# qwagrox/field-coverage-path-planning

Measured on AMD Instinct MI355X. Metric: validated path points/sec (Clothoid+speed+geofence) on 500x200m field batch, higher is better.
Workload: dtype f64; 1 GPU; cfg1 x 4096: 4096 fields of 500 x 200 m per GPU, ARC turns (the reference's own model, pinned to its outputs) at the reference's sampling, 1691 points per field; a step = one fresh plan call of the ba; turn_model=arc (reference, pinned), points_per_gpu_step=6926336, fields_per_gpu=4096, setup=device

## Files before the change

### field_coverage_path_planning_amd/csrc/fcpp_quiet_fn.h

```cpp
#pragma once
#include "fcpp_pointfn.h"

namespace fcpp {

#ifndef FCPP_DENSE_NT
#define FCPP_DENSE_NT 0
#endif
typedef double st_pair_f64 __attribute__((ext_vector_type(2), aligned(8)));
typedef uint32_t st_pair_u32 __attribute__((ext_vector_type(2), aligned(4)));
template <bool NT>
__device__ __forceinline__ void st2(double *ptr, double a, double b)
{
    st_pair_f64 v = { a, b };
    if (NT) __builtin_nontemporal_store(v, reinterpret_cast<st_pair_f64 *>(ptr));
    else *reinterpret_cast<st_pair_f64 *>(ptr) = v;
}
template <bool NT>
__device__ __forceinline__ void st2(uint32_t *ptr, uint32_t a, uint32_t b)
{
    st_pair_u32 v = { a, b };
    if (NT) __builtin_nontemporal_store(v, reinterpret_cast<st_pair_u32 *>(ptr));
    else *reinterpret_cast<st_pair_u32 *>(ptr) = v;
}
template <bool NT>
__device__ __forceinline__ void store_pair(bool has0, bool has1, int64_t g, double px0, double px1, double py0, double py1, double k0,
                                           double k1, double v, uint32_t f0, uint32_t f1, double *__restrict__ xo,
                                           double *__restrict__ yo, double *__restrict__ ko, double *__restrict__ vo,
                                           uint32_t *__restrict__ fso)
{
    if (has0 && has1) {
        st2<NT>(xo + g, px0, px1);
        st2<NT>(yo + g, py0, py1);
        st2<NT>(ko + g, k0, k1);
        st2<NT>(vo + g, v, v);
        st2<NT>(fso + g, f0, f1);
    } else if (has0) {
        xo[g] = px0; yo[g] = py0; ko[g] = k0; vo[g] = v; fso[g] = f0;
    } else if (has1) {
        xo[g + 1] = px1; yo[g + 1] = py1; ko[g + 1] = k1; vo[g + 1] = v; fso[g + 1] = f1;
    }
}

__device__ __forceinline__ double line_start_curvature(const DevField &q, const DevConst &cst, int idx, double &jump_len)
{
    const int per = q.n_line + q.n_turn;
    double tx, ty, x0, y0, x1, y1;
    uint32_t fw;
    eval_main(q, cst, idx - 1, per - 1, tx, ty, fw);
    eval_main(q, cst, idx, 0, x0, y0, fw);
    eval_main(q, cst, idx, 1, x1, y1, fw);
    const double dx1 = x0 - tx, dy1 = y0 - ty, dx2 = x1 - x0, dy2 = y1 - y0;
    jump_len = seg_len(dx1, dy1);
    return curv_chords(dx1, dy1, jump_len, dx2, dy2, seg_len(dx2, dy2));
}

__device__ __forceinline__ void stage_turn_template(const DevConst &cst, double *__restrict__ tmpl_lds)
{
    const int lane = threadIdx.x & 63;
    if (lane < cst.tmpl_n) {
        const double2 t = cst.tmpl_u[lane];
        tmpl_lds[lane] = t.x; tmpl_lds[TMPL_LDS + lane] = t.y; tmpl_lds[2 * TMPL_LDS + lane] = cst.tmpl_u_dk[lane].y;
    }
    wave_sync();
}

template <int KINDS, bool STAGED, bool OBS>
__device__ __forceinline__ void quiet_tile(const DevTile &tl, const DevField *__restrict__ fg, const DevPrim *__restrict__ prims,
                                           const DevConst &cst, const DevObstacles &obs, double *my_lds ,
                                           double *__restrict__ tmpl_lds ,
                                           double *__restrict__ xo, double *__restrict__ yo, double *__restrict__ ko,
                                           double *__restrict__ vo, uint32_t *__restrict__ fso,
                                           unsigned long long *sink_outside, unsigned long long *sink_obstacle)
{
    const int lane = threadIdx.x & 63;
    const DevField &q = *fg;
    const int cnt = tl.count;
    const int64_t g0 = q.pt_off + tl.start;
    const int odd = (int)(g0 & 1);
    constexpr bool NT = FCPP_DENSE_NT && KINDS != 16;
    const double ntol = -cst.geofence_tol;
    auto outside = [&](double px, double py) -> bool {
        bool out = false;
#pragma unroll
        for (int e = 0; e < 4; ++e) out = out | (q.ex[e] * px + q.ey[e] * py + q.eo[e] < ntol);
        return out;
    };
    int nout = 0, nobs = 0;
    if ((KINDS & 16) && (KINDS == 16 || tl.quiet == 4)) {
        int per = q.n_line + q.n_turn, nl = q.n_line, last = q.n_turn - 1, n_pass = q.P, idx_base = tl.idx0;
        int rev = q.reverse_order, sfr = q.start_from_right, rotated = q.rotated;
        const bool arc = q.turn_model == FCPP_TURN_ARC;
        double xr = arc ? q.max_x : (q.max_x - q.R), xl = arc ? q.min_x : (q.min_x + q.R);
        double k_last = cst.turn_kappa_last[q.reverse_order ? 1 : 0];
        double k_start = cst.field_junc[tl.field].x;
        double min_y = q.min_y, Wd = q.W, lstep = q.line_step, lex = q.lex, lsx = q.lsx;
        double rc = q.rot_cos, rs = q.rot_sin, rcx = q.rot_cx, rcy = q.rot_cy;
        double v_work = cst.v_work, v_turn = cst.v_turn;
        double e0x = q.ex[0], e0y = q.ey[0], e0o = q.eo[0], e1x = q.ex[1], e1y = q.ey[1], e1o = q.eo[1];
        double e2x = q.ex[2], e2y = q.ey[2], e2o = q.eo[2], e3x = q.ex[3], e3y = q.ey[3], e3o = q.eo[3];
        double ntl = ntol;
        int n_obs = q.obs_count;
        const bool fence = q.span_inside == 0;
        FCPP_PIN(per); FCPP_PIN(nl); FCPP_PIN(last); FCPP_PIN(n_pass); FCPP_PIN(idx_base); FCPP_PIN(rev); FCPP_PIN(sfr); FCPP_PIN(rotated);
        FCPP_PIN(xr); FCPP_PIN(xl); FCPP_PIN(k_last); FCPP_PIN(k_start); FCPP_PIN(min_y); FCPP_PIN(Wd); FCPP_PIN(lstep); FCPP_PIN(lex); FCPP_PIN(lsx);
        FCPP_PIN(v_work); FCPP_PIN(v_turn); FCPP_PIN(n_obs);
        FCPP_PIN_V(rc); FCPP_PIN_V(rs); FCPP_PIN_V(rcx); FCPP_PIN_V(rcy);
        FCPP_PIN_V(e0x); FCPP_PIN_V(e0y); FCPP_PIN_V(e0o); FCPP_PIN_V(e1x); FCPP_PIN_V(e1y); FCPP_PIN_V(e1o);
        FCPP_PIN_V(e2x); FCPP_PIN_V(e2y); FCPP_PIN_V(e2o); FCPP_PIN_V(e3x); FCPP_PIN_V(e3y); FCPP_PIN_V(e3o); FCPP_PIN_V(ntl);
        auto outside_s = [&](double px, double py) -> bool {
            return (e0x * px + e0y * py + e0o < ntl) | (e1x * px + e1y * py + e1o < ntl) | (e2x * px + e2y * py + e2o < ntl) |
                   (e3x * px + e3y * py + e3o < ntl);
        };
        auto sample = [&](int dq, int off, double &px, double &py, double &kp, double &v, uint32_t &fw) {
            const int idx = idx_base + dq;
            const int pi = rev ? (n_pass - 1 - idx) : idx;
            const double y = min_y + (double)pi * Wd;
            const bool go_left = sfr ? ((idx & 1) == 0) : ((idx & 1) == 1);
            if (off < nl) {
                px = go_left ? ((double)off * -lstep + lex) : ((double)off * lstep + lsx);
                if (off == nl - 1) px = go_left ? lsx : lex;
                py = y;
                kp = (off == 0 && idx > 0) ? k_start : 0.0;
                v = v_work;
                fw = FCPP_KIND_SWATH | ((uint32_t)pi << FCPP_INDEX_SHIFT);
            } else {
                const int c = off - nl;
                double tx, ty, tk;
                if (STAGED) { tx = tmpl_lds[c]; ty = tmpl_lds[TMPL_LDS + c]; tk = tmpl_lds[2 * TMPL_LDS + c]; }
                else { const double2 t = cst.tmpl_u[c]; tx = t.x; ty = t.y; tk = cst.tmpl_u_dk[c].y; }
                const bool turn_right = !go_left;
                px = arc ? (turn_right ? (xr - tx) : (xl + tx)) : (turn_right ? (xr + tx) : (xl - tx));
                py = y + ty;
                kp = c == last ? k_last : tk;
                v = v_turn;
                fw = FCPP_KIND_UTURN | ((uint32_t)pi << FCPP_INDEX_SHIFT);
            }
            if (rotated) {
                const double tx = px - rcx, ty = py - rcy;
                px = (tx * rc - ty * rs) + rcx;
                py = (tx * rs + ty * rc) + rcy;
            }
        };
        const unsigned uper = (unsigned)per, step_q = 128u / uper, step_r = 128u - step_q * uper;
        const unsigned a1 = (unsigned)(tl.off0 + 2 * lane - odd + 1);
        int dq1 = (int)(a1 / uper), off1 = (int)(a1 - (unsigned)dq1 * uper);
#pragma unroll
        for (int k = 0; k < TILE_POINTS / 128; ++k) {
            if (k > 0 && 128 * k - odd >= cnt) break;
            const int j = 2 * (lane + 64 * k) - odd;
            const bool has0 = j >= 0 && j < cnt, has1 = j + 1 < cnt;
            double px0, py0, k0, v0, px1, py1, k1, v1;
            uint32_t f0, f1;
            const int dq0 = off1 == 0 ? dq1 - 1 : dq1, off0 = off1 == 0 ? per - 1 : off1 - 1;
            sample(dq0, off0, px0, py0, k0, v0, f0);
            sample(dq1, off1, px1, py1, k1, v1, f1);
            off1 += (int)step_r; dq1 += (int)step_q;
            if (off1 >= per) { off1 -= per; ++dq1; }
            if (fence) {
                const bool o0 = has0 && outside_s(px0, py0), o1 = has1 && outside_s(px1, py1);
                nout += (o0 ? 1 : 0) + (o1 ? 1 : 0);
                f0 |= o0 ? FCPP_FLAG_OUTSIDE : 0u;
                f1 |= o1 ? FCPP_FLAG_OUTSIDE : 0u;
            }
            if (OBS && n_obs > 0) {
                double mnx = has0 ? px0 : (has1 ? px1 : FCPP_INF), mxx = has0 ? px0 : (has1 ? px1 : -FCPP_INF);
                double mny = has0 ? py0 : (has1 ? py1 : FCPP_INF), mxy = has0 ? py0 : (has1 ? py1 : -FCPP_INF);
                if (has1) { mnx = fmin(mnx, px1); mxx = fmax(mxx, px1); mny = fmin(mny, py1); mxy = fmax(mxy, py1); }
#pragma unroll
                for (int o = 32; o > 0; o >>= 1) {
                    mnx = fmin(mnx, __shfl_xor(mnx, o)); mny = fmin(mny, __shfl_xor(mny, o));
                    mxx = fmax(mxx, __shfl_xor(mxx, o)); mxy = fmax(mxy, __shfl_xor(mxy, o));
                }
                const double ox[2] = { has0 ? px0 : px1, px1 }, oy[2] = { has0 ? py0 : py1, py1 };
                const unsigned m = obstacle_mask<2>(obs, q.obs_first, q.obs_first + q.obs_count, my_lds, mnx, mny, mxx, mxy, ox, oy,
                                                    has1 ? 2 : (has0 ? 1 : 0));
                const bool b0 = has0 && (m & 1u), b1 = has1 && (m & 2u);
                nobs += (b0 ? 1 : 0) + (b1 ? 1 : 0);
                f0 |= b0 ? FCPP_FLAG_OBSTACLE : 0u;
                f1 |= b1 ? FCPP_FLAG_OBSTACLE : 0u;
            }
            const int64_t g = g0 + j;
            if (has0 && has1) {
                st2<NT>(xo + g, px0, px1);
                st2<NT>(yo + g, py0, py1);
                st2<NT>(ko + g, k0, k1);
                st2<NT>(vo + g, v0, v1);
                st2<NT>(fso + g, f0, f1);
            } else if (has0) {
                xo[g] = px0; yo[g] = py0; ko[g] = k0; vo[g] = v0; fso[g] = f0;
            } else if (has1) {
                xo[g + 1] = px1; yo[g + 1] = py1; ko[g + 1] = k1; vo[g + 1] = v1; fso[g + 1] = f1;
            }
        }
    } else if ((KINDS & 8) && (KINDS == 8 || tl.quiet == 3)) {
        const int idx = tl.idx0;
        const int pi = q.reverse_order ? (q.P - 1 - idx) : idx;
        const double y = q.min_y + (double)pi * q.W;
        const bool go_left = q.start_from_right ? ((idx & 1) == 0) : ((idx & 1) == 1);
        const bool turn_right = !go_left, arc = q.turn_model == FCPP_TURN_ARC;
        const double xr = arc ? q.max_x : (q.max_x - q.R), xl = arc ? q.min_x : (q.min_x + q.R);
        const uint32_t fw = FCPP_KIND_UTURN | ((uint32_t)pi << FCPP_INDEX_SHIFT);
        const double k_last = cst.turn_kappa_last[q.reverse_order ? 1 : 0];
        const int last = q.n_turn - 1;
        auto sample = [&](int tk, double &px, double &py, double &kp) {
            const int c = min(max(tk, 0), last);
            const double2 t = cst.tmpl_u[c];
            px = arc ? (turn_right ? (xr - t.x) : (xl + t.x)) : (turn_right ? (xr + t.x) : (xl - t.x));
            py = y + t.y;
            if (q.rotated) rotate_back(q, px, py);
            kp = c == last ? k_last : cst.tmpl_u_dk[c].y;
        };
#pragma unroll
        for (int k = 0; k < TILE_POINTS / 128; ++k) {
            if (k > 0 && 128 * k - odd >= cnt) break;
            const int j = 2 * (lane + 64 * k) - odd;
            const bool has0 = j >= 0 && j < cnt, has1 = j + 1 < cnt;
            double px0, py0, k0, px1, py1, k1;
            sample(tl.off0 + j, px0, py0, k0);
            sample(tl.off0 + j + 1, px1, py1, k1);
            uint32_t f0 = fw, f1 = fw;
            const bool o0 = has0 && outside(px0, py0), o1 = has1 && outside(px1, py1);
            nout += (o0 ? 1 : 0) + (o1 ? 1 : 0);
            f0 |= o0 ? FCPP_FLAG_OUTSIDE : 0u;
            f1 |= o1 ? FCPP_FLAG_OUTSIDE : 0u;
            if (OBS && q.obs_count > 0) {
                double mnx = has0 ? px0 : (has1 ? px1 : FCPP_INF), mxx = has0 ? px0 : (has1 ? px1 : -FCPP_INF);
                double mny = has0 ? py0 : (has1 ? py1 : FCPP_INF), mxy = has0 ? py0 : (has1 ? py1 : -FCPP_INF);
                if (has1) { mnx = fmin(mnx, px1); mxx = fmax(mxx, px1); mny = fmin(mny, py1); mxy = fmax(mxy, py1); }
#pragma unroll
                for (int o = 32; o > 0; o >>= 1) {
                    mnx = fmin(mnx, __shfl_xor(mnx, o)); mny = fmin(mny, __shfl_xor(mny, o));
                    mxx = fmax(mxx, __shfl_xor(mxx, o)); mxy = fmax(mxy, __shfl_xor(mxy, o));
                }
                const double ox[2] = { has0 ? px0 : px1, px1 }, oy[2] = { has0 ? py0 : py1, py1 };
                const unsigned m = obstacle_mask<2>(obs, q.obs_first, q.obs_first + q.obs_count, my_lds, mnx, mny, mxx, mxy, ox, oy,
                                                    has1 ? 2 : (has0 ? 1 : 0));
                const bool b0 = has0 && (m & 1u), b1 = has1 && (m & 2u);
                nobs += (b0 ? 1 : 0) + (b1 ? 1 : 0);
                f0 |= b0 ? FCPP_FLAG_OBSTACLE : 0u;
                f1 |= b1 ? FCPP_FLAG_OBSTACLE : 0u;
            }
            store_pair<NT>(has0, has1, g0 + j, px0, px1, py0, py1, k0, k1, cst.v_turn, f0, f1, xo, yo, ko, vo, fso);
        }
    } else if (KINDS & 6) {
        double ax, ay, sx, sy, bx, by, vnom;
        int n_lin;
        uint32_t fw;
        bool rot;
        if (tl.quiet == 1) {
            const int idx = tl.idx0;
            const int pi = q.reverse_order ? (q.P - 1 - idx) : idx;
            const bool go_left = q.start_from_right ? ((idx & 1) == 0) : ((idx & 1) == 1);
            ax = go_left ? q.lex : q.lsx; bx = go_left ? q.lsx : q.lex; sx = go_left ? -q.line_step : q.line_step;
            ay = by = q.min_y + (double)pi * q.W; sy = 0.0;
            n_lin = q.n_line;
            rot = q.rotated != 0;
            fw = FCPP_KIND_SWATH | ((uint32_t)pi << FCPP_INDEX_SHIFT);
            vnom = cst.v_work;
        } else {
            const DevPrim &p = prims[tl.idx0];
            ax = p.a[0]; ay = p.a[1]; bx = p.a[2]; by = p.a[3]; sx = p.a[4]; sy = p.a[5];
            n_lin = p.n;
            rot = false;
            fw = p.fs; vnom = p.v_nom;
        }
        auto lin = [&](int r, double &px, double &py) {
            px = (double)r * sx + ax; py = (double)r * sy + ay;
            if (r == n_lin - 1) { px = bx; py = by; }
        };
        const bool has_start = tl.quiet == 1 && tl.off0 == 0 && tl.idx0 > 0;
        const double k_start = has_start ? cst.field_junc[tl.field].x : 0.0;
        double ex0, ey0, ex1, ey1;
        lin(tl.off0, ex0, ey0);
        lin(tl.off0 + cnt - 1, ex1, ey1);
        if (rot) { rotate_back(q, ex0, ey0); rotate_back(q, ex1, ey1); }
        const bool ends_out = outside(ex0, ey0) || outside(ex1, ey1);
        const double bminx = fmin(ex0, ex1), bmaxx = fmax(ex0, ex1), bminy = fmin(ey0, ey1), bmaxy = fmax(ey0, ey1);
#pragma unroll
        for (int k = 0; k < TILE_POINTS / 128; ++k) {
            if (k > 0 && 128 * k - odd >= cnt) break;
            const int j = 2 * (lane + 64 * k) - odd;
            const bool has0 = j >= 0 && j < cnt, has1 = j + 1 < cnt;
            double px0, py0, px1, py1;
            lin(tl.off0 + j, px0, py0);
            lin(tl.off0 + j + 1, px1, py1);
            if (rot) { rotate_back(q, px0, py0); rotate_back(q, px1, py1); }
            uint32_t f0 = fw, f1 = fw;
            if (ends_out) {
                const bool o0 = has0 && outside(px0, py0), o1 = has1 && outside(px1, py1);
                nout += (o0 ? 1 : 0) + (o1 ? 1 : 0);
                f0 |= o0 ? FCPP_FLAG_OUTSIDE : 0u;
                f1 |= o1 ? FCPP_FLAG_OUTSIDE : 0u;
            }
            if (OBS && q.obs_count > 0) {
                const double ox[2] = { has0 ? px0 : px1, px1 }, oy[2] = { has0 ? py0 : py1, py1 };
                const unsigned m = obstacle_mask<2>(obs, q.obs_first, q.obs_first + q.obs_count, my_lds, bminx, bminy, bmaxx, bmaxy,
                                                    ox, oy, has1 ? 2 : (has0 ? 1 : 0));
                const bool b0 = has0 && (m & 1u), b1 = has1 && (m & 2u);
                nobs += (b0 ? 1 : 0) + (b1 ? 1 : 0);
                f0 |= b0 ? FCPP_FLAG_OBSTACLE : 0u;
                f1 |= b1 ? FCPP_FLAG_OBSTACLE : 0u;
            }
            const double k0 = (has_start && j == 0) ? k_start : 0.0, k1 = (has_start && j + 1 == 0) ? k_start : 0.0;
            store_pair<NT>(has0, has1, g0 + j, px0, px1, py0, py1, k0, k1, vnom, f0, f1, xo, yo, ko, vo, fso);
        }
    }
    if (__ballot(nout | nobs)) {
        const long long io = wave_sum_i(nout), ib = wave_sum_i(nobs);
        if (lane == 0 && io) atomicAdd(sink_outside, (unsigned long long)io);
        if (lane == 0 && ib) atomicAdd(sink_obstacle, (unsigned long long)ib);
    }
}

struct FieldStatView {
    int n_line, n_turn, reverse_order;
    double line_step;
    int64_t n_main;
    double2 junc;
    __device__ __forceinline__ void set(const DevField &q, double2 j) { n_line = q.n_line; n_turn = q.n_turn; reverse_order = q.reverse_order; line_step = q.line_step; n_main = q.n_main; junc = j; }
    __device__ __forceinline__ void load(const DevField *__restrict__ fields, const DevConst &cst, int64_t field)
    {
        const DevField &q = fields[field];
        n_line = q.n_line; n_turn = q.n_turn; reverse_order = q.reverse_order; line_step = q.line_step; n_main = q.n_main;
        junc = cst.field_junc ? cst.field_junc[field] : make_double2(0.0, 0.0);
    }
};

__device__ __forceinline__ TilePartial quiet_run_partial(const DevRun &run, const DevTile &tl, const FieldStatView &q,
                                                         const DevPrim *__restrict__ prims, const DevConst &cst)
{
    TilePartial tp;
    tp.main_len = tp.main_time_pre = tp.main_time = tp.head_len = tp.head_time_pre = tp.head_time = 0.0;
    tp.max_kappa = tp.max_alat = tp.max_jump = 0.0;
    tp.n_viol = 0; tp.n_outside = 0; tp.n_in_obstacle = 0; tp.n_adjusted = 0;
    if (tl.quiet == 4) {
        const bool rv = q.reverse_order != 0;
        const double tmk = rv ? cst.turn_max_kappa[1] : cst.turn_max_kappa[0], tmj = rv ? cst.turn_max_jump[1] : cst.turn_max_jump[0];
        const double tkl = rv ? cst.turn_kappa_last[1] : cst.turn_kappa_last[0];
        const int per = q.n_line + q.n_turn;
        const double n_pass = (double)(run.count / per), n_jump = n_pass - (tl.idx0 == 0 ? 1.0 : 0.0);
        const double line_len = (double)(q.n_line - 1) * fabs(q.line_step);
        const double2 junc = q.junc;
        const double jl = n_jump > 0.0 ? junc.y : 0.0, k0 = n_jump > 0.0 ? junc.x : 0.0;
        tp.main_len = n_pass * (line_len + cst.turn_len) + n_jump * jl;
        tp.main_time_pre = tp.main_time = n_pass * (line_len / fmax(cst.ms_work, 0.1) + cst.turn_time) +
                                          n_jump * (jl / fmax(((cst.v_turn + cst.v_work) / 2) / 3.6, 0.1));
        tp.max_kappa = fmax(tmk, k0);
        tp.max_alat = fmax(cst.ms_turn * cst.ms_turn * tmk, cst.ms_work * cst.ms_work * k0);
        tp.max_jump = fmax(tmj, n_jump > 0.0 ? fmax(fabs(k0 - tkl), k0) : 0.0);
    } else     if (tl.quiet == 3) {
        const bool rv = q.reverse_order != 0;
        const double tmk = rv ? cst.turn_max_kappa[1] : cst.turn_max_kappa[0];
        tp.main_len = cst.turn_len; tp.main_time_pre = tp.main_time = cst.turn_time;
        tp.max_kappa = tmk; tp.max_alat = cst.ms_turn * cst.ms_turn * tmk;
        tp.max_jump = rv ? cst.turn_max_jump[1] : cst.turn_max_jump[0];
    } else {
        double step_len, msnom;
        int layer;
        if (tl.quiet == 1) { step_len = fabs(q.line_step); msnom = cst.ms_work; layer = 0; }
        else {
            const DevPrim &p = prims[tl.idx0];
            const double sx = p.a[4], sy = p.a[5];
            step_len = (sy == 0.0) ? fabs(sx) : ((sx == 0.0) ? fabs(sy) : sqrt(sx * sx + sy * sy));
            msnom = nominal_ms(p.fs, cst); layer = tl.start >= q.n_main ? 1 : 0;
        }
        const bool at_line_start = tl.quiet == 1 && tl.off0 == 0;
        double len = (double)(at_line_start ? run.count - 1 : run.count) * step_len, t = len / fmax(msnom, 0.1);
        if (at_line_start && tl.idx0 > 0) {
            const double k0 = q.junc.x, jl = q.junc.y;
            len += jl;
            t += jl / fmax(((cst.v_turn + cst.v_work) / 2) / 3.6, 0.1);
            tp.max_kappa = k0; tp.max_alat = cst.ms_work * cst.ms_work * k0;
            tp.max_jump = fmax(fabs(k0 - (q.reverse_order ? cst.turn_kappa_last[1] : cst.turn_kappa_last[0])), k0);
        }
        tp.main_len = layer ? 0.0 : len; tp.main_time_pre = layer ? 0.0 : t; tp.main_time = layer ? 0.0 : t;
        tp.head_len = layer ? len : 0.0; tp.head_time_pre = layer ? t : 0.0; tp.head_time = layer ? t : 0.0;
    }
    return tp;
}

}
```

### field_coverage_path_planning_amd/csrc/fcpp_sparse.hip

```cpp
#include "fcpp_sparse2_fn.h"
#include "fcpp_quiet_fn.h"
#include "fcpp_devplan.h"

namespace fcpp {

template <int SP_WAVES, int PTS>
__global__ __launch_bounds__(64 * SP_WAVES) void k_plan_sparse(const DevWaveTile *__restrict__ wtiles, const int32_t *__restrict__ ids, int64_t n_wtiles,
                                                               const DevField *__restrict__ fields, const DevPrim *__restrict__ prims,
                                                               DevConst cst, DevObstacles obs, double *__restrict__ xo, double *__restrict__ yo,
                                                               double *__restrict__ ko, double *__restrict__ vo, uint32_t *__restrict__ fso,
                                                               TilePartial *__restrict__ partial, int xcd_map)
{
    __shared__ double obs_lds[SP_WAVES][2 * OBS_LDS_VERTS];
    __shared__ double atab[ATAN_TAB_DOUBLES];
    __shared__ double plds[SP_WAVES][TILE_PRIMS_LDS];
    const int wave = __builtin_amdgcn_readfirstlane((int)(threadIdx.x >> 6)), lane = threadIdx.x & 63;
    const unsigned bid = xcd_map ? (blockIdx.x & 7u) * (gridDim.x >> 3) + (blockIdx.x >> 3) : blockIdx.x;
    const int64_t slot = (int64_t)bid * SP_WAVES + wave;
    if (slot >= n_wtiles) return;
    atan_tab_stage(atab);
    const DevWaveTile wt = wtiles[ids ? (int64_t)ids[slot] : slot];
    SparseAcc acc;
    acc.clear();
    sparse_tile2<false>(wt, fields[wt.field], prims, cst, obs, obs_lds[wave], atab, plds[wave], xo, yo, ko, vo, fso, acc);

    double g[3] = { 0.0, 0.0, 0.0 };
    const int out0 = wt.hb, out1 = wt.hb + wt.count;
    if (out0 < wt.rel_seam) g[0] = wave4_to_hi<0>(acc.s_len[0], acc.s_tpre[0], acc.s_t[0], 0.0);
    if (out1 > wt.rel_seam + 1) g[1] = wave4_to_hi<0>(acc.s_len[1], acc.s_tpre[1], acc.s_t[1], 0.0);
    if (__ballot(acc.mk != 0.0 || acc.mj != 0.0) != 0ull) g[2] = wave4_to_hi<1>(acc.mk, acc.ma, acc.mj, 0.0);
    const int vs = WAVE4_SLOT(lane);
    if (lane >= 60 && vs < 3) {
        double *tp = reinterpret_cast<double *>(&partial[wt.tile]);
        tp[vs] = g[0]; tp[3 + vs] = g[1]; tp[6 + vs] = g[2];
    }
    if (lane == 63) {
        TilePartial &tp = partial[wt.tile];
        tp.n_viol = acc.c_viol; tp.n_outside = acc.c_out; tp.n_in_obstacle = acc.c_obs; tp.n_adjusted = acc.c_adj;
    }
}

template <int W, bool OBS>
__device__ __forceinline__ void field_span_chunk(const DevFieldPack &pk, int wave, const DevConst &cst, const DevObstacles &obs, double *obs_lds,
                                                 double *tlds, double *__restrict__ xo, double *__restrict__ yo, double *__restrict__ ko,
                                                 double *__restrict__ vo, uint32_t *__restrict__ fso, unsigned long long *cnt)
{
    static_assert(W == FUSED_SPAN_CHUNKS, "one chunk per wavefront");
    const int64_t S = pk.span_points;
    const DevField &f = pk.field;
    const unsigned per = (unsigned)(f.n_line + f.n_turn);
    const int r0 = (int)(f.pt_off & (TILE_POINTS - 1));
    const int c_first = (int)(S < TILE_POINTS - r0 ? S : TILE_POINTS - r0);
    const int n_chunks = (int)((r0 + S + TILE_POINTS - 1) / TILE_POINTS);
    if (wave >= n_chunks) return;
    wave_sync();
    stage_turn_template(cst, tlds);
    DevTile tl;
    const unsigned start = wave == 0 ? 0u : (unsigned)(c_first + (wave - 1) * TILE_POINTS);
    tl.field = pk.work.field; tl.start = start; tl.quiet = 4; tl.stat_tile = 0;
    tl.count = wave == 0 ? c_first : (int)((S - start < TILE_POINTS) ? S - start : TILE_POINTS);
    tl.idx0 = __builtin_amdgcn_readfirstlane((int)(start / per)); tl.off0 = __builtin_amdgcn_readfirstlane((int)(start - (unsigned)tl.idx0 * per));
    tl.count = __builtin_amdgcn_readfirstlane(tl.count);
    quiet_tile<16, true, OBS>(tl, &f, nullptr, cst, obs, obs_lds, tlds, xo, yo, ko, vo, fso, cnt, cnt + 1);
}

struct DirectRule {
    int64_t n = 0, gen = 0;
    const int64_t *plan_totals = nullptr, *agg = nullptr;
};
template <int W, bool OBS, bool SPANS, bool DIRECT = false>
__device__ __forceinline__ void plan_sparse_fields_body(const DevFieldPack *__restrict__ packs,
                                                              DevConst cst, double *__restrict__ xo, double *__restrict__ yo,
                                                              double *__restrict__ ko, double *__restrict__ vo, uint32_t *__restrict__ fso,
                                                              DevObstacles obs, TilePartial *__restrict__ partial,
                                                              const TilePartial *__restrict__ totals, fcpp_field_stats *__restrict__ stats,
                                                              const DirectRule rule = DirectRule())
{
    __shared__ double obs_lds[W][OBS ? 2 * OBS_LDS_VERTS : 1];
    __shared__ TilePartial red[FIELD_WORK_TILES];
    __shared__ double atab[ATAN_TAB_DOUBLES];
    static_assert(3 * TMPL_LDS >= TILE_PRIMS_LDS, "one area serves both phases");
    __shared__ double wlds[W][3 * TMPL_LDS];
    __shared__ unsigned long long span_cnt[W][2];
    const int wave = __builtin_amdgcn_readfirstlane((int)(threadIdx.x >> 6)), lane = threadIdx.x & 63;
    atan_tab_stage(atab);
    const unsigned wg = DIRECT ? blockIdx.x - 1u : blockIdx.x;
    const DevFieldPack &pk = packs[wg];
    const DevFieldWork w = pk.work;
    if (DIRECT) {
        int64_t flag[PF_COUNT];
#pragma unroll
        for (int k = 0; k < PF_COUNT; ++k) flag[k] = rule.plan_totals[PC_COLS + k];
        const int nblk = (int)offset_blocks(rule.n);
        const int64_t a_work = offset_total_part(rule.agg, nblk, PC_WORK, lane), a_unf = offset_total_part(rule.agg, nblk, PC_UNFUSABLE, lane),
                      a_wsp = offset_total_part(rule.agg, nblk, PC_WORK_SPAN_PTS, lane);
        bool ok = off_wave_sum(a_work) == rule.n && off_wave_sum(a_unf) == 0 && off_wave_sum(a_wsp) > 0;
#pragma unroll
        for (int k = 0; k < PF_COUNT; ++k) ok = ok && flag[k] != rule.gen;
        if (!ok || w.n_tiles < 0) return;
        __builtin_amdgcn_sched_barrier(0);
    }
#ifdef FCPP_DIAG_SPARSE
    if (g_sparse_stop == -2) return;
#endif
    auto plan_tile = [&](const int t) {
        const DevWaveTile wt = pk.tile[t];
        SparseAcc acc;
        acc.clear();
        sparse_tile2<true>(wt, pk.field, pk.prims[t], cst, obs, obs_lds[wave], atab, wlds[wave], xo, yo, ko, vo, fso, acc);
        double g[3] = { 0.0, 0.0, 0.0 };
        const int out0 = wt.hb, out1 = wt.hb + wt.count;
        if (out0 < wt.rel_seam) g[0] = wave4_to_hi<0>(acc.s_len[0], acc.s_tpre[0], acc.s_t[0], 0.0);
        if (out1 > wt.rel_seam + 1) g[1] = wave4_to_hi<0>(acc.s_len[1], acc.s_tpre[1], acc.s_t[1], 0.0);
        if (__ballot(acc.mk != 0.0 || acc.mj != 0.0) != 0ull) g[2] = wave4_to_hi<1>(acc.mk, acc.ma, acc.mj, 0.0);
        const int vs = WAVE4_SLOT(lane);
        if (lane >= 60 && vs < 3) {
            double *tp = reinterpret_cast<double *>(&red[t]);
            tp[vs] = g[0]; tp[3 + vs] = g[1]; tp[6 + vs] = g[2];
        }
        if (lane == 63) { red[t].n_viol = acc.c_viol; red[t].n_outside = acc.c_out; red[t].n_in_obstacle = acc.c_obs; red[t].n_adjusted = acc.c_adj; }
    };
    if (lane < 2) span_cnt[wave][lane] = 0;
    auto span_phase = [&]() {
        const DevFieldPack *pk2 = &pk;
        asm volatile("" : "+s"(pk2) : : "memory");
        if (pk2->span_points > 0) field_span_chunk<W, OBS>(*pk2, wave, cst, obs, obs_lds[wave], wlds[wave], xo, yo, ko, vo, fso, &span_cnt[wave][0]);
    };
    if (wave < w.n_tiles) plan_tile(wave);
    if (SPANS) span_phase();
    static_assert(sizeof(TilePartial) == 13 * 8 && sizeof(fcpp_field_stats) == 13 * 8, "statistics records are thirteen 8-byte components");
    unsigned long long run_v = 0, c_out = 0, c_obs = 0;
    if (wave == 0) {
        if (lane < 13) run_v = reinterpret_cast<const unsigned long long *>(&totals[wg])[lane];
        if (!DIRECT && lane < w.n_entries) { const TilePartial &slot = partial[w.e_first + lane]; c_out = (unsigned long long)slot.n_outside; c_obs = (unsigned long long)slot.n_in_obstacle; }
    }
    asm volatile("s_waitcnt lgkmcnt(0)\n\ts_barrier" ::: "memory");
    if (wave != 0) return;
    if (!DIRECT && (c_out | c_obs) != 0ull) { partial[w.e_first + lane].n_outside = 0; partial[w.e_first + lane].n_in_obstacle = 0; }
    if (lane < W) { c_out += span_cnt[lane][0]; c_obs += span_cnt[lane][1]; }
    if (__ballot((c_out | c_obs) != 0ull) != 0ull) {
#pragma unroll
        for (int o = FIELD_WORK_ENTRIES / 2; o > 0; o >>= 1) { c_out += __shfl_xor(c_out, o); c_obs += __shfl_xor(c_obs, o); }
    }
    if (lane >= 13) return;
    const unsigned long long *rv = reinterpret_cast<const unsigned long long *>(red) + lane;
    unsigned long long bits;
    if (lane < 9) {
        double a = __longlong_as_double((long long)run_v);
        for (int t = 0; t < w.n_tiles; ++t) {
            const double x = __longlong_as_double((long long)rv[13 * t]);
            a = lane < 6 ? a + x : max_raw(a, x);
        }
        bits = (unsigned long long)__double_as_longlong(a);
    } else {
        bits = run_v;
        for (int t = 0; t < w.n_tiles; ++t) bits += rv[13 * t];
        if (lane == 10) bits += c_out;
        if (lane == 11) bits += c_obs;
    }
    reinterpret_cast<unsigned long long *>(&stats[w.field])[lane] = bits;
}

template <int W, bool OBS, bool SPANS>
__global__ __launch_bounds__(64 * W) void k_plan_sparse_fields(const DevFieldPack *__restrict__ packs, DevConst cst, double *__restrict__ xo, double *__restrict__ yo,
                                                              double *__restrict__ ko, double *__restrict__ vo, uint32_t *__restrict__ fso,
                                                              DevObstacles obs, TilePartial *__restrict__ partial,
                                                              const TilePartial *__restrict__ totals, fcpp_field_stats *__restrict__ stats)
{
    plan_sparse_fields_body<W, OBS, SPANS>(packs, cst, xo, yo, ko, vo, fso, obs, partial, totals, stats);
}

template <int W>
__global__ __launch_bounds__(64 * W) void k_plan_sparse_fields_direct(const DevFieldPack *__restrict__ packs, DevConst cst, double *__restrict__ xo, double *__restrict__ yo,
                                                                     double *__restrict__ ko, double *__restrict__ vo, uint32_t *__restrict__ fso,
                                                                     const TilePartial *__restrict__ totals, fcpp_field_stats *__restrict__ stats, int64_t n, int64_t gen,
                                                                     int64_t *__restrict__ plan_totals, const int64_t *__restrict__ agg, int64_t *__restrict__ agg_next,
                                                                     int64_t *__restrict__ mirror)
{
    if (blockIdx.x == 0) {
        publish_two_level(n, gen, plan_totals, agg, agg_next, mirror, __builtin_amdgcn_readfirstlane((int)(threadIdx.x >> 6)), (int)(threadIdx.x & 63));
        return;
    }
    DevObstacles obs = { nullptr, nullptr, nullptr, nullptr };
    DirectRule rule;
    rule.n = n; rule.gen = gen; rule.plan_totals = plan_totals; rule.agg = agg;
    plan_sparse_fields_body<W, false, true, true>(packs, cst, xo, yo, ko, vo, fso, obs, nullptr, totals, stats, rule);
}

__global__ void k_work_totals(int64_t n_work, const DevFieldWork *__restrict__ work, const int64_t *__restrict__ stat_run,
                              const TilePartial *__restrict__ partial, TilePartial *__restrict__ totals)
{
    const int64_t i = (int64_t)blockIdx.x * blockDim.x + threadIdx.x;
    if (i >= n_work) return;
    const DevFieldWork w = work[i];
    TilePartial t;
    memset(&t, 0, sizeof t);
    for (int e = 0; e < w.n_entries; ++e) {
        if (stat_run[w.e_first + e] == 0) continue;
        const TilePartial p = partial[w.e_first + e];
        t.main_len += p.main_len; t.main_time_pre += p.main_time_pre; t.main_time += p.main_time;
        t.head_len += p.head_len; t.head_time_pre += p.head_time_pre; t.head_time += p.head_time;
        t.max_kappa = fmax(t.max_kappa, p.max_kappa); t.max_alat = fmax(t.max_alat, p.max_alat); t.max_jump = fmax(t.max_jump, p.max_jump);
        t.n_viol += p.n_viol; t.n_adjusted += p.n_adjusted;
    }
    totals[i] = t;
}

int launch_work_totals(hipStream_t st, int64_t n_work, const DevFieldWork *work, const int64_t *stat_run, const TilePartial *partial, TilePartial *totals)
{
    if (n_work <= 0) return 0;
    hipLaunchKernelGGL(k_work_totals, dim3((unsigned)((n_work + 255) / 256)), dim3(256), 0, st, n_work, work, stat_run, partial, totals);
    hipError_t e = hipGetLastError();
    return e == hipSuccess ? 0 : (int)e;
}

int launch_plan_sparse_fields(hipStream_t st, int64_t n_work, const DevFieldPack *packs, const DevConst &cst, const DevObstacles &obs, double *x,
                              double *y, double *kappa, double *v, uint32_t *fs, TilePartial *partial, int waves, const TilePartial *totals,
                              fcpp_field_stats *stats, bool spans)
{
    if (n_work <= 0) return 0;
#define FCPP_FW(K, W, OB, SP) FCPP_LAUNCH((K<W, OB, SP>), dim3((unsigned)n_work), dim3(64 * W), 0, st, packs, cst, x, y, kappa, v, fs, obs, partial, totals, stats)
    if (waves != 4) return (int)hipErrorInvalidValue;
    const bool has_obs = obs.offsets != nullptr;
    if (has_obs && spans) FCPP_FW(k_plan_sparse_fields, 4, true, true);
    else if (has_obs) FCPP_FW(k_plan_sparse_fields, 4, true, false);
    else if (spans) FCPP_FW(k_plan_sparse_fields, 4, false, true);
    else FCPP_FW(k_plan_sparse_fields, 4, false, false);
#undef FCPP_FW
    hipError_t e = hipGetLastError();
    return e == hipSuccess ? 0 : (int)e;
}

int launch_plan_sparse_direct(hipStream_t st, int64_t n, int64_t gen, const DevPlanScratch &s, const DevConst &cst, double *x, double *y, double *kappa,
                              double *v, uint32_t *fs, fcpp_field_stats *stats, int64_t *totals_host)
{
    if (n <= 0) return 0;
    if (n > OFF_FIELDS_MAX || !s.direct_packs || !s.agg || !s.agg_next || !totals_host) return (int)hipErrorInvalidValue;
    DevConst dc = cst;
    dc.field_junc = s.direct_junc;
    FCPP_LAUNCH((k_plan_sparse_fields_direct<4>), dim3((unsigned)n + 1u), dim3(64 * 4), 0, st, s.direct_packs, dc, x, y, kappa, v, fs, s.direct_totals, stats, n, gen,
                s.totals, s.agg, s.agg_next, totals_host);
    hipError_t e = hipGetLastError();
    return e == hipSuccess ? 0 : (int)e;
}

int launch_plan_sparse(hipStream_t st, int64_t n_wtiles, const DevWaveTile *wtiles, const DevField *fields, const DevPrim *prims,
                       const DevConst &cst, const DevObstacles &obs, double *x, double *y, double *kappa, double *v, uint32_t *fs,
                       TilePartial *partial, const int32_t *ids)
{
    if (n_wtiles <= 0) return 0;
    auto grid8 = [&](int64_t per) { const int64_t g = (n_wtiles + per - 1) / per; return dim3((unsigned)((g + 7) / 8 * 8)); };
    if (n_wtiles >= 65536) FCPP_LAUNCH((k_plan_sparse<2, 2>), grid8(2), dim3(128), 0, st, wtiles, ids, n_wtiles, fields, prims, cst, obs, x, y, kappa, v, fs, partial, 1);
    else FCPP_LAUNCH((k_plan_sparse<4, 2>), grid8(4), dim3(256), 0, st, wtiles, ids, n_wtiles, fields, prims, cst, obs, x, y, kappa, v, fs, partial, 1);
    hipError_t e = hipGetLastError();
    return e == hipSuccess ? 0 : (int)e;
}

}

#ifdef FCPP_DIAG_SPARSE
extern "C" long long fcpp_diag_sparse(unsigned *rows, long long cap)
{
    unsigned n = 0, zero = 0;
    if (hipDeviceSynchronize() != hipSuccess) return -1;
    if (hipMemcpyFromSymbol(&n, HIP_SYMBOL(fcpp::g_sparse_diag_next), sizeof n) != hipSuccess) return -1;
    const long long m = n < (unsigned)fcpp::SP_DIAG_SLOTS ? n : fcpp::SP_DIAG_SLOTS;
    const long long c = m < cap ? m : cap;
    if (c > 0 && hipMemcpyFromSymbol(rows, HIP_SYMBOL(fcpp::g_sparse_diag), (size_t)c * 16 * sizeof(unsigned)) != hipSuccess) return -1;
    if (hipMemcpyToSymbol(HIP_SYMBOL(fcpp::g_sparse_diag_next), &zero, sizeof zero) != hipSuccess) return -1;
    return n;
}
extern "C" int fcpp_diag_sparse_stop(int section)
{
    return hipMemcpyToSymbol(HIP_SYMBOL(fcpp::g_sparse_stop), &section, sizeof section) == hipSuccess ? 0 : -1;
}
#endif
```

### field_coverage_path_planning_amd/csrc/fcpp_sparse_fn.h

```cpp
#pragma once
#include "fcpp_pointfn.h"

namespace fcpp {

struct SparseAcc {
    double s_len[2], s_tpre[2], s_t[2], mk, ma, mj;
    int c_viol, c_out, c_obs, c_adj;
    __device__ __forceinline__ void clear()
    {
        s_len[0] = s_len[1] = s_tpre[0] = s_tpre[1] = s_t[0] = s_t[1] = mk = ma = mj = 0.0;
        c_viol = c_out = c_obs = c_adj = 0;
    }
};

static constexpr int TILE_PRIMS_MAX = 9, PRIM_DOUBLES = (int)(sizeof(DevPrim) / sizeof(double)), TILE_STARTS_AT = TILE_PRIMS_MAX * PRIM_DOUBLES + 1,
                     TILE_PRIMS_LDS = TILE_STARTS_AT + 5;
static_assert(sizeof(DevPrim) % sizeof(double) == 0 && TILE_PRIMS_MAX * PRIM_DOUBLES <= 128, "two loads per lane stage a tile's primitives");
__device__ __forceinline__ void tile_slots2(const DevWaveTile &wt, int lane, int &sa, int &sb)
{
    unsigned long long mlo = 0, mhi = 0;
#pragma unroll
    for (int k = 0; k < 8; ++k) {
        const unsigned t = wt.thr[k];
        if (t < 64u) mlo |= 1ull << t;
        else if (t < 128u) mhi |= 1ull << (t - 64u);
    }
    const bool hi = lane >= 32;
    const unsigned long long m = hi ? mhi : mlo;
    const int p = (2 * lane) & 63;
    sa = __popcll(m & ((2ull << p) - 1ull)) + (hi ? __popcll(mlo) : 0);
    sb = sa + (int)((m >> (p + 1)) & 1ull);
}

template <bool PACKED = false>
__device__ __forceinline__ void stage_tile_prims(const DevWaveTile &wt, const DevPrim *__restrict__ prims, double *plds, int nl)
{
    const int lane = threadIdx.x & 63;
    if (PACKED) {
        const double *src = reinterpret_cast<const double *>(prims);
        const double v0 = src[lane], v1 = lane + 64 < TILE_PRIMS_MAX * PRIM_DOUBLES ? src[lane + 64] : 0.0;
        plds[lane] = v0;
        if (lane + 64 < TILE_PRIMS_MAX * PRIM_DOUBLES) plds[lane + 64] = v1;
    } else {
        if (wt.rel_main >= nl) return;
        int np = 1;
#pragma unroll
        for (int k = 0; k < 8; ++k) np += wt.thr[k] != 255 ? 1 : 0;
        const double *src = reinterpret_cast<const double *>(prims + wt.p0);
        const int nw = np * PRIM_DOUBLES;
        if (lane < nw) plds[lane] = src[lane];
        if (lane + 64 < nw) plds[lane + 64] = src[lane + 64];
    }
    if (lane < TILE_PRIMS_MAX) {
        const unsigned long long th = (unsigned long long)wt.thr[0] | (unsigned long long)wt.thr[1] << 8 | (unsigned long long)wt.thr[2] << 16 |
                                      (unsigned long long)wt.thr[3] << 24 | (unsigned long long)wt.thr[4] << 32 | (unsigned long long)wt.thr[5] << 40 |
                                      (unsigned long long)wt.thr[6] << 48 | (unsigned long long)wt.thr[7] << 56;
        reinterpret_cast<int *>(plds + TILE_STARTS_AT)[lane] = lane == 0 ? -wt.r0 : (int)((th >> (8 * (lane - 1))) & 255ull);
    }
    wave_sync();
}

}
```

Before: 55.06 billion points/s.

## Prefetch per-pack primitives, turn template, and totals into LDS at kernel entry

The fused field kernel now issues its global loads for tile primitives, the turn template, field junction curvature, running totals and partial counters up front, before the DIRECT flag wait, and stores them into dedicated LDS areas. Each load's latency can then overlap the flag polling and other setup instead of sitting on the critical path inside each phase. The span phase copies the field struct from constant address space, and reads k_start from LDS rather than from global memory. In exchange the kernel uses more LDS (separate prim and template areas) and more registers, which could lower occupancy. Some loads are also issued for workgroups that later exit early.

```diff
diff --git a/field_coverage_path_planning_amd/csrc/fcpp_quiet_fn.h b/field_coverage_path_planning_amd/csrc/fcpp_quiet_fn.h
--- a/field_coverage_path_planning_amd/csrc/fcpp_quiet_fn.h
+++ b/field_coverage_path_planning_amd/csrc/fcpp_quiet_fn.h
@@ -63,6 +63,16 @@
     }
     wave_sync();
 }
+__device__ __forceinline__ void load_turn_template(const DevConst &cst, int lane, double2 &t, double &k)
+{
+    t = make_double2(0.0, 0.0);
+    k = 0.0;
+    if (lane < cst.tmpl_n) { t = cst.tmpl_u[lane]; k = cst.tmpl_u_dk[lane].y; }
+}
+__device__ __forceinline__ void keep_turn_template(const DevConst &cst, int lane, double *__restrict__ tmpl_lds, double2 t, double k)
+{
+    if (lane < cst.tmpl_n) { tmpl_lds[lane] = t.x; tmpl_lds[TMPL_LDS + lane] = t.y; tmpl_lds[2 * TMPL_LDS + lane] = k; }
+}
 
 template <int KINDS, bool STAGED, bool OBS>
 __device__ __forceinline__ void quiet_tile(const DevTile &tl, const DevField *__restrict__ fg, const DevPrim *__restrict__ prims,
@@ -70,7 +80,8 @@
                                            double *__restrict__ tmpl_lds ,
                                            double *__restrict__ xo, double *__restrict__ yo, double *__restrict__ ko,
                                            double *__restrict__ vo, uint32_t *__restrict__ fso,
-                                           unsigned long long *sink_outside, unsigned long long *sink_obstacle)
+                                           unsigned long long *sink_outside, unsigned long long *sink_obstacle,
+                                           const double *k_start_lds = nullptr)
 {
     const int lane = threadIdx.x & 63;
     const DevField &q = *fg;
@@ -92,7 +103,7 @@
         const bool arc = q.turn_model == FCPP_TURN_ARC;
         double xr = arc ? q.max_x : (q.max_x - q.R), xl = arc ? q.min_x : (q.min_x + q.R);
         double k_last = cst.turn_kappa_last[q.reverse_order ? 1 : 0];
-        double k_start = cst.field_junc[tl.field].x;
+        double k_start = k_start_lds ? *k_start_lds : cst.field_junc[tl.field].x;
         double min_y = q.min_y, Wd = q.W, lstep = q.line_step, lex = q.lex, lsx = q.lsx;
         double rc = q.rot_cos, rs = q.rot_sin, rcx = q.rot_cx, rcy = q.rot_cy;
         double v_work = cst.v_work, v_turn = cst.v_turn;
diff --git a/field_coverage_path_planning_amd/csrc/fcpp_sparse.hip b/field_coverage_path_planning_amd/csrc/fcpp_sparse.hip
--- a/field_coverage_path_planning_amd/csrc/fcpp_sparse.hip
+++ b/field_coverage_path_planning_amd/csrc/fcpp_sparse.hip
@@ -40,28 +40,40 @@
     }
 }
 
+
+typedef const DevField __attribute__((address_space(4))) ConstField;
+__device__ __forceinline__ void copy_const_field(DevField &f, ConstField *c)
+{
+    static_assert(sizeof(DevField) == 312, "every member is copied below");
+    f.pt_off = c->pt_off; f.n_main = c->n_main; f.gen_main = c->gen_main; f.n_total = c->n_total;
+    f.lsx = c->lsx; f.lex = c->lex; f.line_step = c->line_step; f.min_x = c->min_x; f.max_x = c->max_x; f.min_y = c->min_y;
+    f.W = c->W; f.R = c->R; f.turn_step = c->turn_step; f.turn_end = c->turn_end; f.turn_Re = c->turn_Re;
+    f.rot_cos = c->rot_cos; f.rot_sin = c->rot_sin; f.rot_cx = c->rot_cx; f.rot_cy = c->rot_cy; f.v_work = c->v_work; f.v_turn = c->v_turn;
+    f.P = c->P; f.n_line = c->n_line; f.n_turn = c->n_turn; f.reverse_order = c->reverse_order; f.start_from_right = c->start_from_right;
+    f.rotated = c->rotated; f.turn_model = c->turn_model; f.prim_first = c->prim_first; f.prim_count = c->prim_count;
+    f.obs_first = c->obs_first; f.obs_count = c->obs_count; f.span_inside = c->span_inside;
+#pragma unroll
+    for (int e = 0; e < 4; ++e) { f.ex[e] = c->ex[e]; f.ey[e] = c->ey[e]; f.eo[e] = c->eo[e]; }
+}
+
 template <int W, bool OBS>
-__device__ __forceinline__ void field_span_chunk(const DevFieldPack &pk, int wave, const DevConst &cst, const DevObstacles &obs, double *obs_lds,
-                                                 double *tlds, double *__restrict__ xo, double *__restrict__ yo, double *__restrict__ ko,
+__device__ __forceinline__ void field_span_chunk(const int64_t S, const int field, const DevField &f, int wave, const DevConst &cst, const DevObstacles &obs, double *obs_lds,
+                                                 double *tlds, const double *k_start_lds, double *__restrict__ xo, double *__restrict__ yo, double *__restrict__ ko,
                                                  double *__restrict__ vo, uint32_t *__restrict__ fso, unsigned long long *cnt)
 {
     static_assert(W == FUSED_SPAN_CHUNKS, "one chunk per wavefront");
-    const int64_t S = pk.span_points;
-    const DevField &f = pk.field;
     const unsigned per = (unsigned)(f.n_line + f.n_turn);
     const int r0 = (int)(f.pt_off & (TILE_POINTS - 1));
     const int c_first = (int)(S < TILE_POINTS - r0 ? S : TILE_POINTS - r0);
     const int n_chunks = (int)((r0 + S + TILE_POINTS - 1) / TILE_POINTS);
     if (wave >= n_chunks) return;
-    wave_sync();
-    stage_turn_template(cst, tlds);
     DevTile tl;
     const unsigned start = wave == 0 ? 0u : (unsigned)(c_first + (wave - 1) * TILE_POINTS);
-    tl.field = pk.work.field; tl.start = start; tl.quiet = 4; tl.stat_tile = 0;
+    tl.field = field; tl.start = start; tl.quiet = 4; tl.stat_tile = 0;
     tl.count = wave == 0 ? c_first : (int)((S - start < TILE_POINTS) ? S - start : TILE_POINTS);
     tl.idx0 = __builtin_amdgcn_readfirstlane((int)(start / per)); tl.off0 = __builtin_amdgcn_readfirstlane((int)(start - (unsigned)tl.idx0 * per));
     tl.count = __builtin_amdgcn_readfirstlane(tl.count);
-    quiet_tile<16, true, OBS>(tl, &f, nullptr, cst, obs, obs_lds, tlds, xo, yo, ko, vo, fso, cnt, cnt + 1);
+    quiet_tile<16, true, OBS>(tl, &f, nullptr, cst, obs, obs_lds, tlds, xo, yo, ko, vo, fso, cnt, cnt + 1, k_start_lds);
 }
 
 struct DirectRule {
@@ -79,14 +91,26 @@
     __shared__ double obs_lds[W][OBS ? 2 * OBS_LDS_VERTS : 1];
     __shared__ TilePartial red[FIELD_WORK_TILES];
     __shared__ double atab[ATAN_TAB_DOUBLES];
-    static_assert(3 * TMPL_LDS >= TILE_PRIMS_LDS, "one area serves both phases");
-    __shared__ double wlds[W][3 * TMPL_LDS];
+    constexpr int JUNC_AT = 3 * TMPL_LDS;
+    __shared__ double plds[W][TILE_PRIMS_LDS];
+    __shared__ double tlds[W][SPANS ? JUNC_AT + 1 : 1];
+    __shared__ unsigned long long run_lds[13], cnt_lds[DIRECT ? 1 : FIELD_WORK_ENTRIES][2];
     __shared__ unsigned long long span_cnt[W][2];
     const int wave = __builtin_amdgcn_readfirstlane((int)(threadIdx.x >> 6)), lane = threadIdx.x & 63;
     atan_tab_stage(atab);
     const unsigned wg = DIRECT ? blockIdx.x - 1u : blockIdx.x;
     const DevFieldPack &pk = packs[wg];
+    static_assert(W <= FIELD_WORK_TILES, "a wavefront's primitive slots are the pack's");
+    static_assert(sizeof(TilePartial) == 13 * 8 && sizeof(fcpp_field_stats) == 13 * 8, "statistics records are thirteen 8-byte components");
+    double pv0, pv1, tk = 0.0;
+    double2 tu = make_double2(0.0, 0.0), junc = make_double2(0.0, 0.0);
+    unsigned long long run_v = 0, c_out = 0, c_obs = 0;
+    load_tile_prims(pk.prims[wave], lane, pv0, pv1);
+    if (SPANS) load_turn_template(cst, lane, tu, tk);
+    if (wave == 0 && lane < 13) run_v = reinterpret_cast<const unsigned long long *>(&totals[wg])[lane];
+    if (SPANS && DIRECT) junc = cst.field_junc[wg];
     const DevFieldWork w = pk.work;
+    const int64_t span_points = SPANS ? pk.span_points : 0;
     if (DIRECT) {
         int64_t flag[PF_COUNT];
 #pragma unroll
@@ -100,6 +124,18 @@
         if (!ok || w.n_tiles < 0) return;
         __builtin_amdgcn_sched_barrier(0);
     }
+    if (SPANS && !DIRECT && span_points > 0) junc = cst.field_junc[w.field];
+    if (!DIRECT && wave == 0 && lane < w.n_entries) { const TilePartial &slot = partial[w.e_first + lane]; c_out = (unsigned long long)slot.n_outside; c_obs = (unsigned long long)slot.n_in_obstacle; }
+    keep_tile_prims(plds[wave], lane, pv0, pv1);
+    if (SPANS) {
+        keep_turn_template(cst, lane, tlds[wave], tu, tk);
+        if (lane == 0) tlds[wave][JUNC_AT] = junc.x;
+    }
+    if (wave == 0) {
+        if (lane < 13) run_lds[lane] = run_v;
+        if (!DIRECT && lane < FIELD_WORK_ENTRIES) { cnt_lds[lane][0] = c_out; cnt_lds[lane][1] = c_obs; }
+    }
+    wave_sync();
 #ifdef FCPP_DIAG_SPARSE
     if (g_sparse_stop == -2) return;
 #endif
@@ -107,7 +143,7 @@
         const DevWaveTile wt = pk.tile[t];
         SparseAcc acc;
         acc.clear();
-        sparse_tile2<true>(wt, pk.field, pk.prims[t], cst, obs, obs_lds[wave], atab, wlds[wave], xo, yo, ko, vo, fso, acc);
+        sparse_tile2<true>(wt, pk.field, nullptr, cst, obs, obs_lds[wave], atab, plds[wave], xo, yo, ko, vo, fso, acc);
         double g[3] = { 0.0, 0.0, 0.0 };
         const int out0 = wt.hb, out1 = wt.hb + wt.count;
         if (out0 < wt.rel_seam) g[0] = wave4_to_hi<0>(acc.s_len[0], acc.s_tpre[0], acc.s_t[0], 0.0);
@@ -124,18 +160,19 @@
     auto span_phase = [&]() {
         const DevFieldPack *pk2 = &pk;
         asm volatile("" : "+s"(pk2) : : "memory");
-        if (pk2->span_points > 0) field_span_chunk<W, OBS>(*pk2, wave, cst, obs, obs_lds[wave], wlds[wave], xo, yo, ko, vo, fso, &span_cnt[wave][0]);
+        typedef const DevFieldPack __attribute__((address_space(4))) ConstPack;
+        if (span_points <= 0) return;
+        DevField f;
+        copy_const_field(f, &((ConstPack *)pk2)->field);
+        field_span_chunk<W, OBS>(span_points, w.field, f, wave, cst, obs, obs_lds[wave], tlds[wave], &tlds[wave][JUNC_AT], xo, yo, ko, vo, fso, &span_cnt[wave][0]);
     };
     if (wave < w.n_tiles) plan_tile(wave);
     if (SPANS) span_phase();
-    static_assert(sizeof(TilePartial) == 13 * 8 && sizeof(fcpp_field_stats) == 13 * 8, "statistics records are thirteen 8-byte components");
-    unsigned long long run_v = 0, c_out = 0, c_obs = 0;
-    if (wave == 0) {
-        if (lane < 13) run_v = reinterpret_cast<const unsigned long long *>(&totals[wg])[lane];
-        if (!DIRECT && lane < w.n_entries) { const TilePartial &slot = partial[w.e_first + lane]; c_out = (unsigned long long)slot.n_outside; c_obs = (unsigned long long)slot.n_in_obstacle; }
-    }
     asm volatile("s_waitcnt lgkmcnt(0)\n\ts_barrier" ::: "memory");
     if (wave != 0) return;
+    run_v = lane < 13 ? run_lds[lane] : 0ull;
+    c_out = c_obs = 0;
+    if (!DIRECT && lane < FIELD_WORK_ENTRIES) { c_out = cnt_lds[lane][0]; c_obs = cnt_lds[lane][1]; }
     if (!DIRECT && (c_out | c_obs) != 0ull) { partial[w.e_first + lane].n_outside = 0; partial[w.e_first + lane].n_in_obstacle = 0; }
     if (lane < W) { c_out += span_cnt[lane][0]; c_obs += span_cnt[lane][1]; }
     if (__ballot((c_out | c_obs) != 0ull) != 0ull) {
diff --git a/field_coverage_path_planning_amd/csrc/fcpp_sparse_fn.h b/field_coverage_path_planning_amd/csrc/fcpp_sparse_fn.h
--- a/field_coverage_path_planning_amd/csrc/fcpp_sparse_fn.h
+++ b/field_coverage_path_planning_amd/csrc/fcpp_sparse_fn.h
@@ -32,11 +32,23 @@
     sb = sa + (int)((m >> (p + 1)) & 1ull);
 }
 
+__device__ __forceinline__ void load_tile_prims(const DevPrim *__restrict__ prims, int lane, double &v0, double &v1)
+{
+    const double *src = reinterpret_cast<const double *>(prims);
+    v0 = src[lane];
+    v1 = lane + 64 < TILE_PRIMS_MAX * PRIM_DOUBLES ? src[lane + 64] : 0.0;
+}
+__device__ __forceinline__ void keep_tile_prims(double *plds, int lane, double v0, double v1)
+{
+    plds[lane] = v0;
+    if (lane + 64 < TILE_PRIMS_MAX * PRIM_DOUBLES) plds[lane + 64] = v1;
+}
 template <bool PACKED = false>
 __device__ __forceinline__ void stage_tile_prims(const DevWaveTile &wt, const DevPrim *__restrict__ prims, double *plds, int nl)
 {
     const int lane = threadIdx.x & 63;
-    if (PACKED) {
+    if (PACKED && prims == nullptr) {
+    } else if (PACKED) {
         const double *src = reinterpret_cast<const double *>(prims);
         const double v0 = src[lane], v1 = lane + 64 < TILE_PRIMS_MAX * PRIM_DOUBLES ? src[lane + 64] : 0.0;
         plds[lane] = v0;
```

After: 54.88 billion points/s. No clear change (-0.3%).
